# AtomGradient/swift-qwen3-tts

Hardware: AMD Instinct MI355X
Metric: codec_tokens_per_s (higher is better)
Workload: dtype bf16

## Files before the change

### swift-qwen3-tts_amd/csrc/debug_env.cc

```cpp
#include <atomic>
#include <cstdlib>
#include <mutex>

#include "kernels.h"

namespace q3 {

namespace {
std::mutex g_mu;
std::atomic<const DebugEnv*> g_env{nullptr};

bool flag(const char* name) { return std::getenv(name) != nullptr; }
int number(const char* name, int dflt) {
    const char* e = std::getenv(name);
    return e && *e ? std::atoi(e) : dflt;
}

const DebugEnv* read_env() {
    DebugEnv* d = new DebugEnv{};
    d->gemm_no_row_split = flag("Q3TTS_GEMM_NO_ROW_SPLIT");
    d->gemm_one_pair = flag("Q3TTS_GEMM_ONE_PAIR");
    d->no_tall_gemm = flag("Q3TTS_NO_TALL_GEMM");
    d->tall_shape = number("Q3TTS_TALL_SHAPE", 0);
    d->chunk_qsplit = number("Q3TTS_CHUNK_QSPLIT", 0);
    d->conv_no_pw = flag("Q3TTS_CONV_NO_PW");
    d->nt_off = std::getenv("Q3TTS_NT") && number("Q3TTS_NT", 1) == 0;
    d->serial_jobs = number("Q3TTS_SERIAL_JOBS", 0) != 0;
    d->fail_back_half = number("Q3TTS_TEST_FAIL_BACK_HALF", 0) != 0;
    d->no_prefix_cache = number("Q3TTS_NO_PREFIX_CACHE", 0) != 0;
    return d;
}
}

const DebugEnv& debug_env() {
    const DebugEnv* e = g_env.load(std::memory_order_acquire);
    if (!e) {
        std::lock_guard<std::mutex> lk(g_mu);
        e = g_env.load(std::memory_order_acquire);
        if (!e) {
            e = read_env();
            g_env.store(e, std::memory_order_release);
        }
    }
    return *e;
}

void debug_env_reload() {
    std::lock_guard<std::mutex> lk(g_mu);
    g_env.store(read_env(), std::memory_order_release);
}

}
```

### swift-qwen3-tts_amd/csrc/engine.cc

```cpp
#include "engine.h"

#include <algorithm>
#include <cctype>
#include <chrono>
#include <cmath>
#include <cstdio>
#include <deque>
#include <functional>
#include <thread>

#include "codec.h"
#include "frontend.h"

namespace q3 {

namespace {
std::string lower(const std::string& s) {
    std::string o = s;
    for (auto& c : o) c = char(std::tolower((unsigned char)c));
    return o;
}
const char* const kCodecRangeMsg =
    "Audio decoding failed: the codec decoder produced a non-finite waveform -- also on the fp32 matrix-core convolutions (the "
    "reference's range), which a row is re-decoded on when it leaves the fp16 range of the default two-plane kernels";
// ... 235 lines not shown
        compose_b_ = nullptr;
        if (!pass) {
            ws_bytes_ = align_up(b.off, 256);
            Q3_HIP(hipMalloc(reinterpret_cast<void**>(&ws_), ws_bytes_));
            Q3_HIP(hipMemset(ws_, 0, ws_bytes_));
        }
    }
    std::vector<int32_t> cbt((size_t)(Bm_));
    for (int i = 0; i < Bm_; ++i) cbt[size_t(i)] = i;
    Q3_HIP(hipMemcpy(cp_block_table_, cbt.data(), cbt.size() * 4, hipMemcpyHostToDevice));
}

GemmArgs Engine::gemm_args(const LinearW& L, const uint16_t* x, int M) const {
    GemmArgs a{};
    a.W = L.w;
    a.Wsb = L.sb;
    a.x = x;
    a.xMB = Mp_ / 16;
    a.M = M;
    a.Mpad = int(align_up(size_t(M), 16));
    a.N = L.Np;
    a.K = L.Kp;
    a.bias = L.bias;
    a.ss_ld = Mp_;
    return a;
}

void Engine::enqueue_layers(const StackW& s, Stream& w, int B, uint16_t* kpool, uint16_t* vpool, size_t layer_stride,
                            const int32_t* block_table, int max_pages, const int32_t* kv_len, const uint8_t* active,
                            int ss_count_in, int fixed_len, int chunk, const int32_t* chunk_n_prompt, int chunk_r_base) {
    const int H = s.hidden, MBL = Mp_ / 16, tiles = H / 16;
    const int M = B * (chunk > 1 ? chunk : 1);
    Q3_CHECK(M <= Mp_, 7, "internal error: chunk does not fit the activation buffers");
    const bool row_norm = M > 64;
    const bool prologue_qkv = H <= 2048 && !row_norm, prologue_mlp = H <= 2048 && !row_norm;
    const bool nt_off = debug_env().nt_off;
    const bool is_talker = &s == &m_->talker;
    const int ntw = is_talker && !nt_off ? 1 : 0;
    const int ntkv = ntw;
    auto norm_into_xn = [&](const uint16_t* nw, const float* ss, int ss_count) {
        NormRowsArgs n{};
        n.h = w.h; n.hMB = MBL; n.w = nw; n.eps = s.eps; n.out = w.xn; n.outMB = MBL; n.M = M; n.H = H;
        if (row_norm && H <= 2048) { n.ss_in = ss; n.ss_count = ss_count; n.ss_ld = Mp_; }
        launch_norm_rows(n, counted());
    };
    for (size_t l = 0; l < s.layers.size(); ++l) {
        const LayerW& L = s.layers[l];
        if (!prologue_qkv) norm_into_xn(L.ln1, w.ss_a, (l == 0) ? ss_count_in : tiles);
        GemmArgs q = gemm_args(L.qkv, prologue_qkv ? w.h : w.xn, M);
        q.epi = 0; q.y = w.qkv; q.ldy = w.ld_qkv; q.nt_weights = ntw;
        if (prologue_qkv) {
            q.norm_w = L.ln1; q.ss_in = w.ss_a; q.ss_count = (l == 0) ? ss_count_in : tiles; q.norm_dim = H; q.norm_eps = s.eps;
        }
        AttnArgs at{};
        at.qkv = w.qkv; at.ld = w.ld_qkv; at.qn_w = L.qn; at.kn_w = L.kn; at.eps = s.eps;
        at.rope_cos = s.rope_cos; at.rope_sin = s.rope_sin;
        at.kpool = kpool + l * layer_stride; at.vpool = vpool + l * layer_stride;
        at.block_table = block_table; at.max_pages = max_pages; at.kv_len = kv_len; at.active = active;
        at.out = w.ao; at.outMB = MBL; at.n_heads = s.n_heads; at.n_kv = s.n_kv; at.B = B;
        at.fixed_len = fixed_len; at.identity_pages = fixed_len >= 0 ? 1 : 0;
        at.chunk = chunk; at.chunk_n_prompt = chunk_n_prompt; at.chunk_r_base = chunk_r_base;
        at.scale = powf(float(kHeadDim), -0.5f);
        at.nt_kv = ntkv;
        launch_gemm_skinny(q, counted());
        launch_attn_decode(at, counted());
        GemmArgs o = gemm_args(L.o, w.ao, M);
        o.epi = 3; o.y = w.h; o.yMB = MBL; o.resid = 1; o.ss_out = w.ss_b; o.nt_weights = ntw;
        launch_gemm_skinny(o, counted());
        if (!prologue_mlp) norm_into_xn(L.ln2, w.ss_b, tiles);
        GemmArgs g = gemm_args(L.gateup, prologue_mlp ? w.h : w.xn, M);
        g.epi = 2; g.y = w.act; g.yMB = MBL; g.nt_weights = ntw;
        if (prologue_mlp) {
            g.norm_w = L.ln2; g.ss_in = w.ss_b; g.ss_count = tiles; g.norm_dim = H; g.norm_eps = s.eps;
        }
        launch_gemm_skinny(g, counted());
        GemmArgs d = gemm_args(L.down, w.act, M);
        d.epi = 3; d.y = w.h; d.yMB = MBL; d.resid = 1; d.ss_out = w.ss_a; d.nt_weights = ntw;
        launch_gemm_skinny(d, counted());
    }
}

void Engine::enqueue_talker_step(int B, bool with_head) {
    (void)with_head;
    enqueue_layers(m_->talker, tk_, B, kpool_, vpool_, kv_layer_stride_, block_table_, max_pages_, kv_len_, active_, 1, -1, 1, nullptr, 0);
}

void Engine::enqueue_cp_pass(int B, bool from_talker, int head, int cp_pos, bool projected) {
    const TalkerConfig& t = m_->cfg.talker;
    const int H = t.hidden_size, CH = m_->cp.hidden, MBL = Mp_ / 16;
    int ss_count = 1;
    auto talker_norm_into = [&](uint16_t* dst, float* ss_out) {
        NormRowsArgs n{};
        n.h = tk_.h; n.hMB = MBL; n.w = m_->talker.final_norm; n.eps = m_->talker.eps;
        n.out = dst; n.outMB = MBL; n.ss_out = ss_out; n.M = B; n.H = H;
        launch_norm_rows(n, counted());
    };
    if (m_->has_cp_proj && projected) {
        ss_count = CH / 16;
    } else if (m_->has_cp_proj) {
        if (from_talker) talker_norm_into(cp_x2_, nullptr);
        GemmArgs p = gemm_args(m_->cp_proj, from_talker ? cp_x2_ : cp_x_, B);
        p.epi = 3; p.y = cp_.h; p.yMB = MBL; p.resid = 0; p.ss_out = cp_.ss_a;
        launch_gemm_skinny(p, counted());
        ss_count = CH / 16;
    } else if (from_talker) {
        talker_norm_into(cp_.h, cp_.ss_a);
    }
    enqueue_layers(m_->cp, cp_, B, cp_kpool_, cp_vpool_, cp_kv_layer_stride_, cp_block_table_, 1, cp_len_, nullptr, ss_count, cp_pos, 1, nullptr, 0);
}

FrameEndArgs Engine::frame_end_args(int B) const {
    const TalkerConfig& t = m_->cfg.talker;
    FrameEndArgs fe{};
    fe.cur_codes = cur_codes_; fe.codec_emb = m_->codec_emb; fe.cp_emb = m_->cp_emb_dev;
    fe.trailing = trailing_; fe.n_trailing = n_trailing_; fe.trailing_idx = trailing_idx_; fe.Tmax = Tcap_;
    fe.tts_pad = tts_pad_; fe.h = tk_.h; fe.hMB = Mp_ / 16; fe.ss_out = tk_.ss_a; fe.H = t.hidden_size; fe.B = B; fe.groups = t.num_code_groups;
    fe.n_frames = n_frames_; fe.max_frames = max_frames_; fe.finished = finished_; fe.active = active_; fe.cp_len = cp_len_;
    fe.text_open = frame_text_open_; fe.starved = frame_text_open_ ? starved_ : nullptr;
    return fe;
}

void Engine::enqueue_frame(int B, const DebugOpts* dbg) {
    struct Count {
        Engine* e;
        int B;
        ~Count() { e->frame_launches_[B] = e->launches_; }
    } count{this, B};
    launches_ = 0;
    const TalkerConfig& t = m_->cfg.talker;
    const int H = t.hidden_size, V = t.vocab_size, Vc = t.cp.vocab_size, CH = t.cp.hidden_size;
    const int groups = t.num_code_groups, MBL = Mp_ / 16;
    stamp(0);
    enqueue_talker_step(B, true);
    stamp(1);
    uint16_t* next_x = m_->has_cp_proj ? cp_x_ : cp_.h;
    float* next_ss = m_->has_cp_proj ? nullptr : cp_.ss_a;
    const bool pair = 2 * B <= Mp_;
    {
        GemmArgs hd = gemm_args(m_->codec_head, tk_.h, B);
        hd.epi = 0; hd.y = tk_.logits; hd.ldy = tk_.ld_logits;
        hd.norm_w = m_->talker.final_norm; hd.ss_in = tk_.ss_a; hd.ss_count = H / 16; hd.norm_dim = H; hd.norm_eps = m_->talker.eps;
        bool rode = false;
        if (pair) {
            NormRowsArgs n{};
            n.h = tk_.h; n.hMB = MBL; n.w = m_->talker.final_norm; n.eps = m_->talker.eps;
            n.out = next_x; n.outMB = MBL; n.ss_out = next_ss; n.M = B; n.H = H;
            rode = launch_gemm_skinny_with_norm_rows(hd, n, st_);
            if (rode) ++launches_;
            else launch_norm_rows(n, counted());
        }
        if (!rode) launch_gemm_skinny(hd, counted());
    }
    SamplerArgs sa{};
    sa.logits = tk_.logits; sa.ldl = tk_.ld_logits; sa.V = V; sa.sp = sp_dev_; sa.is_talker = 1;
    sa.suppress_lo = V - 1024; sa.suppress_hi = V; sa.eos_id = t.codec_eos_token_id;
    sa.seen = seen_; sa.cb = 0; sa.n_frames = n_frames_; sa.max_frames = max_frames_;
    sa.finished = finished_; sa.active = active_; sa.kv_len = kv_len_; sa.advance = 1; sa.advance_gate = active_;
    sa.cur_codes = cur_codes_; sa.codes = codes_; sa.Fmax = Fcap_;
    sa.forced = dbg ? forced_dev_ : nullptr; sa.forced_frames = dbg ? dbg->frames : 0;
    sa.sampled = dbg ? sampled_dev_ : nullptr;
    sa.emb = m_->codec_emb; sa.emb_ld = H; sa.next_MB = MBL; sa.H = H; sa.B = B;
    if (pair) {
        sa.next_x = next_x; sa.next_row0 = B; sa.next_ss = next_ss ? next_ss + B : nullptr;
    } else {
        sa.next_x = m_->has_cp_proj ? cp_x_ : cp_x2_; sa.next_ss = m_->has_cp_proj ? nullptr : cp_ss2_;
    }
    sa.logits_dump = (dbg && dbg->talker_logits) ? tl_dump_ : nullptr; sa.dump_ld = V; sa.dump_off = 0;
    sa.row_key = frame_row_key_;
    if (pair) {
        launch_sampler(sa, counted());
// ... 2565 lines not shown
    qkv.grow(size_t(rows) * ld);
    w.grow(2 * kHeadDim);
    rope.grow(2 * tab);
    kp.grow(pool);
    vp.grow(pool);
    ot.grow(size_t(Mp) * odim);
    ol.grow(size_t(rows) * odim);
    ints.grow(size_t(B) * (2 + d.max_pages));
    act.grow(size_t(B));
    int32_t *kv_len = ints, *n_prompt = kv_len + B, *bt = n_prompt + B;
    Q3_HIP(hipMemset(ints, 0, size_t(B) * (2 + d.max_pages) * 4));
    Q3_HIP(hipMemcpy(qkv, d.qkv, size_t(rows) * ld * 2, hipMemcpyHostToDevice));
    Q3_HIP(hipMemcpy(w, d.qn_w, kHeadDim * 2, hipMemcpyHostToDevice));
    Q3_HIP(hipMemcpy(w + kHeadDim, d.kn_w, kHeadDim * 2, hipMemcpyHostToDevice));
    Q3_HIP(hipMemcpy(rope, d.rope_cos, tab * 2, hipMemcpyHostToDevice));
    Q3_HIP(hipMemcpy(rope + tab, d.rope_sin, tab * 2, hipMemcpyHostToDevice));
    Q3_HIP(hipMemcpy(kp, d.kpool, pool * 2, hipMemcpyHostToDevice));
    Q3_HIP(hipMemcpy(vp, d.vpool, pool * 2, hipMemcpyHostToDevice));
    if (d.kv_len) Q3_HIP(hipMemcpy(kv_len, d.kv_len, size_t(B) * 4, hipMemcpyHostToDevice));
    if (d.chunk_n_prompt) Q3_HIP(hipMemcpy(n_prompt, d.chunk_n_prompt, size_t(B) * 4, hipMemcpyHostToDevice));
    if (d.block_table) Q3_HIP(hipMemcpy(bt, d.block_table, size_t(B) * d.max_pages * 4, hipMemcpyHostToDevice));
    if (d.active) Q3_HIP(hipMemcpy(act, d.active, size_t(B), hipMemcpyHostToDevice));
    Q3_HIP(hipMemset(ot, 0xff, size_t(Mp) * odim * 2));
    AttnArgs at{};
    at.qkv = qkv; at.ld = ld; at.qn_w = w; at.kn_w = w + kHeadDim; at.eps = d.eps;
    at.rope_cos = rope; at.rope_sin = rope + tab;
    at.kpool = kp; at.vpool = vp;
    at.block_table = bt; at.max_pages = d.max_pages; at.kv_len = kv_len; at.active = d.active ? (const uint8_t*)act : nullptr;
    at.out = ot; at.outMB = Mp / 16; at.n_heads = d.n_heads; at.n_kv = d.n_kv; at.B = B;
    at.scale = d.scale;
    at.fixed_len = d.fixed_len; at.identity_pages = d.identity_pages ? 1 : 0;
    at.chunk = d.chunk; at.chunk_n_prompt = d.chunk_n_prompt ? n_prompt : nullptr; at.chunk_r_base = d.chunk_r_base;
    at.nt_kv = d.nt_kv ? 1 : 0;
    launch_attn_decode(at, st_);
    Q3_HIP(hipGetLastError());
    launch_untile_rows(ot, Mp / 16, ol, odim, rows, odim, st_);
    Q3_HIP(hipStreamSynchronize(st_));
    Q3_HIP(hipMemcpy(d.out, ol, size_t(rows) * odim * 2, hipMemcpyDeviceToHost));
    Q3_HIP(hipMemcpy(d.kpool, kp, pool * 2, hipMemcpyDeviceToHost));
    Q3_HIP(hipMemcpy(d.vpool, vp, pool * 2, hipMemcpyDeviceToHost));
}

void Engine::debug_gemm_check(q3tts_gemm_debug& d, GemmArgs& ga, NormRowsArgs& na) {
    static const uint16_t dummy16 = 0;
    static const uint32_t dummy32 = 0;
    d.rode = d.tall = d.tall_shape = d.split = d.mbw = d.nw = d.ch = d.np = d.gx = d.ntw = 0;
    Q3_CHECK(d.mode == 0 || d.mode == 1, 3, "debug_gemm: unknown mode");
    const bool rider = d.mode == 1 || d.rider_M > 0;
    if (rider) {
        Q3_CHECK(d.rider_M >= 1 && d.rider_MB >= 1 && d.rider_MB <= 64 && d.rider_M <= 16 * d.rider_MB, 3, "debug_gemm: rider rows out of range");
        Q3_CHECK(d.rider_H >= 128 && d.rider_H <= 4096 && d.rider_H % 128 == 0, 3, "debug_gemm: rider_H must be a multiple of 128 up to 4096");
        Q3_CHECK(d.geometry_only || (d.rider_h && d.rider_w && d.rider_out), 3, "debug_gemm: null rider argument");
        if (d.rider_ss_in) Q3_CHECK(d.rider_ss_count >= 1 && d.rider_ss_count <= 256, 3, "debug_gemm: at most 256 partial sums of squares per rider row");
        na.hMB = na.outMB = d.rider_MB; na.eps = d.rider_eps; na.M = d.rider_M; na.H = d.rider_H;
        na.ss_count = d.rider_ss_in ? d.rider_ss_count : 0; na.ss_ld = 16 * d.rider_MB;
    }
    if (d.mode == 1) return;
    Q3_CHECK(d.epi == 0 || d.epi == 2 || d.epi == 3, 3, "debug_gemm: unknown epilogue");
    Q3_CHECK(d.M >= 1 && d.M <= 1024, 3, "debug_gemm: M out of range");
    Q3_CHECK(d.K >= 128 && d.K <= 8192 && d.K % 128 == 0, 3, "debug_gemm: K must be a multiple of 128 up to 8192");
    Q3_CHECK(d.N >= 8 && d.N <= 65536 && d.N % (d.epi == 2 ? 8 : 16) == 0, 3, "debug_gemm: N must be a multiple of 16 (epi 2: of 8)");
    const int Mp = int(align_up(size_t(d.M), 16));
    const bool tiled = d.epi != 0 || d.y_tiled;
    Q3_CHECK(d.xMB <= 64 && 16 * d.xMB >= Mp && d.yMB <= 64 && 16 * d.yMB >= Mp && d.ss_ld >= Mp && d.ss_ld <= 4096, 3,
             "debug_gemm: allocation smaller than the padded batch");
    Q3_CHECK(d.y_cols >= d.N && d.y_cols <= d.N + 1024 && d.y_cols % (tiled ? 128 : 8) == 0, 3, "debug_gemm: y_cols");
// ... 96 lines not shown
        for (int part = 0; part < (d.epi == 2 ? 2 : 1); ++part) {
            const void* W = part ? d.W_up : d.W;
            if (d.quant) {
                dWq.grow(size_t(d.N) * d.K / 8);
                Q3_HIP(hipMemcpy(dWq, W, size_t(d.N) * d.K / 8 * 4, hipMemcpyHostToDevice));
                up16(dsc, part ? d.scales_up : d.scales, size_t(d.N) * d.K / 64);
                up16(dbi, part ? d.biases_up : d.biases, size_t(d.N) * d.K / 64);
                launch_tile_int4(dWq, dsc, dbi, d.N, d.K, dWt, dsb, KC, 0, 1, st_, rpt, 8 * part);
            } else {
                up16(dsrc, static_cast<const uint16_t*>(W), size_t(d.N) * d.K);
                launch_tile_weights(dsrc, d.N, d.K, reinterpret_cast<uint16_t*>(static_cast<uint8_t*>(dWt)), KC, 0, 1, st_, rpt, 8 * part);
            }
            Q3_HIP(hipStreamSynchronize(st_));
        }
        if (d.bias) up16(dbias, d.bias, size_t(d.N));
        if (d.norm) {
            up16(dnw, d.norm_w, size_t(d.K));
            dssi.grow(size_t(d.ss_count) * d.ss_ld);
            Q3_HIP(hipMemcpy(dssi, d.ss_in, size_t(d.ss_count) * d.ss_ld * 4, hipMemcpyHostToDevice));
        }
        if (d.ss_out) {
            dsso.grow(n_ss_out);
            Q3_HIP(hipMemcpy(dsso, d.ss_out, n_ss_out * 4, hipMemcpyHostToDevice));
        }
        ga.W = reinterpret_cast<const uint16_t*>(static_cast<uint8_t*>(dWt));
        ga.Wsb = d.quant ? static_cast<uint32_t*>(dsb) : nullptr;
        ga.x = dx; ga.y = dy;
        ga.bias = d.bias ? static_cast<uint16_t*>(dbias) : nullptr;
        ga.norm_w = d.norm ? static_cast<uint16_t*>(dnw) : nullptr;
        ga.ss_in = d.norm ? static_cast<float*>(dssi) : nullptr;
        ga.ss_out = d.ss_out ? static_cast<float*>(dsso) : nullptr;
    }
    bool launched = true;
    if (d.mode == 1) {
        launch_norm_rows(na, st_);
    } else if (rider) {
        launched = launch_gemm_skinny_with_norm_rows(ga, na, st_);
        Q3_CHECK(launched == (d.rode != 0), 7, "debug_gemm: the rider launch disagrees with gemm_norm_rows_rides");
    } else {
        launch_gemm_skinny(ga, st_);
    }
    Q3_HIP(hipGetLastError());
    Q3_HIP(hipStreamSynchronize(st_));
    if (!launched) return;
    if (d.mode == 0) {
        if (tiled) {
            tmp.resize(size_t(yrows) * d.y_cols);
            Q3_HIP(hipMemcpy(tmp.data(), dy, tmp.size() * 2, hipMemcpyDeviceToHost));
            host_untile(tmp, d.y, yrows, d.y_cols);
        } else {
            Q3_HIP(hipMemcpy(d.y, dy, size_t(yrows) * d.y_cols * 2, hipMemcpyDeviceToHost));
        }
        if (d.ss_out) Q3_HIP(hipMemcpy(d.ss_out, dsso, n_ss_out * 4, hipMemcpyDeviceToHost));
    }
    if (rider) {
        tmp.resize(size_t(rrows) * d.rider_H);
        Q3_HIP(hipMemcpy(tmp.data(), rout, tmp.size() * 2, hipMemcpyDeviceToHost));
        host_untile(tmp, d.rider_out, rrows, d.rider_H);
        if (d.rider_ss_out) Q3_HIP(hipMemcpy(d.rider_ss_out, rsso, size_t(rrows) * 4, hipMemcpyDeviceToHost));
    }
}

static void check_caller_codes(const CodecW& w, const int32_t* codes, const int32_t* n_frames, int batch, int max_frames) {
    for (int b = 0; b < batch; ++b)
        for (int f = 0; f < n_frames[b]; ++f) {
            const int32_t* c = codes + (size_t(b) * max_frames + f) * 16;
// ... 669 lines not shown
```

### swift-qwen3-tts_amd/csrc/kernels.h

```cpp
#pragma once
#include <hip/hip_runtime.h>

#include <cstdint>

namespace q3 {

struct DebugEnv {
    bool gemm_no_row_split;
    bool gemm_one_pair;
    bool no_tall_gemm;
    int tall_shape;
    int chunk_qsplit;
    bool conv_no_pw;
    bool nt_off;
    bool serial_jobs;
    bool fail_back_half;
    bool no_prefix_cache;
};
const DebugEnv& debug_env();
void debug_env_reload();

constexpr int kPageTokens = 64;
constexpr int kHeadDim = 128;

struct NormRowsArgs {
    const uint16_t* h;
    int hMB;
    const uint16_t* w;
    float eps;
    uint16_t* out;
    int outMB;
    float* ss_out;
    int M, H;
    const float* ss_in;
    int ss_count, ss_ld;
};
void launch_norm_rows(const NormRowsArgs& a, hipStream_t st);

struct GemmArgs {
    const uint16_t* W;
    const uint32_t* Wsb;
    const uint16_t* x;
    int xMB;
    int M, Mpad, N, K;
    int epi;
    uint16_t* y;
    int ldy;
    int y_tiled, yMB;
    const uint16_t* bias;
    int act_silu;
    const uint16_t* norm_w;
    const float* ss_in;
    int ss_count, ss_ld, norm_dim;
    float norm_eps;
    int nt_weights;
    int resid;
    float* ss_out;
};
void launch_gemm_skinny(const GemmArgs& a, hipStream_t st);
struct SkinnyGeom {
    bool tall;
    int split, mbw;
    int nw, ch, np;
    int gx;
    bool ntw;
};
SkinnyGeom skinny_geometry(const GemmArgs& a);
bool launch_gemm_skinny_with_norm_rows(const GemmArgs& a, const NormRowsArgs& n, hipStream_t st);
bool gemm_norm_rows_rides(const GemmArgs& a, const NormRowsArgs& n);
bool launch_gemm_tall(const GemmArgs& a, hipStream_t st);
bool gemm_tall_takes(const GemmArgs& a);
int gemm_tall_shape(const GemmArgs& a);


struct AttnArgs {
    const uint16_t* qkv;
    int ld;
    const uint16_t* qn_w;
    const uint16_t* kn_w;
    float eps;
    const uint16_t* rope_cos;
    const uint16_t* rope_sin;
    uint16_t* kpool;
// ... 171 lines not shown
```

### swift-qwen3-tts_amd/csrc/kernels/gemm_decode.hip

```cpp
#include "../common.h"
#include "../kernels.h"
#include "row_jobs.h"

namespace q3 {

namespace {

#include "gemm_body.inc"

template <int MB, int EPI, int NW, int CH, bool NORM, bool QUANT, int NP = 1, bool NTW = false>
__global__ __launch_bounds__(NW * 64) void gemm_skinny_kernel(GemmArgs a) {
    __builtin_amdgcn_s_setprio(3);
    gemm_skinny_body<MB, EPI, NW, CH, NORM, QUANT, NP, NTW>(a, blockIdx.x, blockIdx.y * MB);
}

struct GemmSideArgs {
    GemmArgs g;
    NormRowsArgs n;
    int tiles;
};
template <int MB, int CH, bool QUANT>
__global__ __launch_bounds__(512) void gemm_skinny_side_kernel(GemmSideArgs s) {
    __builtin_amdgcn_s_setprio(3);
    if (int(blockIdx.x) >= s.tiles) {
// ... 10 lines not shown
    const dim3 grid(g.gx, g.split);
#define Q3_GEMM(NWv, CHv) \
    hipLaunchKernelGGL((gemm_skinny_kernel<MB, EPI, NWv, CHv, NORM, QUANT, 1, NTW>), grid, dim3(NWv * 64), 0, st, a)
    if constexpr (MB == 4 && !NORM && !NTW) {
        if (g.ch == 0 && g.np == 2) { hipLaunchKernelGGL((gemm_skinny_kernel<4, EPI, 8, 0, false, QUANT, 2, false>), grid, dim3(512), 0, st, a); return; }
        if (g.ch == 0 && g.np == 4) { hipLaunchKernelGGL((gemm_skinny_kernel<4, EPI, 8, 0, false, QUANT, 4, false>), grid, dim3(512), 0, st, a); return; }
    }
    if constexpr (EPI == 2 && MB <= 2) {
        if (g.np > 1) {
#define Q3_GEMM_NP(CHv, NPv) hipLaunchKernelGGL((gemm_skinny_kernel<MB, 2, 8, CHv, NORM, QUANT, NPv, NTW>), grid, dim3(512), 0, st, a)
            if (g.ch == 1) { if (g.np == 2) Q3_GEMM_NP(1, 2); else Q3_GEMM_NP(1, 3); }
            else { if (g.np == 2) Q3_GEMM_NP(2, 2); else Q3_GEMM_NP(2, 3); }
#undef Q3_GEMM_NP
            return;
        }
    }
    if (g.nw == 4) {
        Q3_GEMM(4, 1);
    } else {
        switch (g.ch) {
            case 1: Q3_GEMM(8, 1); break;
            case 2: Q3_GEMM(8, 2); break;
            case 3: Q3_GEMM(8, 3); break;
            case 6: Q3_GEMM(8, 6); break;
            default: Q3_GEMM(8, 0); break;
        }
    }
#undef Q3_GEMM
}

template <int EPI, bool NORM, bool QUANT>
void launch_q(const GemmArgs& a, hipStream_t st) {
    const SkinnyGeom g = skinny_geometry(a);
    if (g.ntw) {
        if (g.mbw == 1) launch_mb<1, EPI, NORM, QUANT, true>(a, g, st);
        else launch_mb<2, EPI, NORM, QUANT, true>(a, g, st);
        return;
    }
    switch (g.mbw) {
        case 1: launch_mb<1, EPI, NORM, QUANT, false>(a, g, st); break;
        case 2: launch_mb<2, EPI, NORM, QUANT, false>(a, g, st); break;
        case 3: launch_mb<3, EPI, NORM, QUANT, false>(a, g, st); break;
        case 4: launch_mb<4, EPI, NORM, QUANT, false>(a, g, st); break;
        default: throw Error(3, "gemm_skinny: more than 4 row blocks per workgroup");
    }
}

template <int EPI, bool NORM>
void launch_epi(const GemmArgs& a, hipStream_t st) {
    if (a.Wsb) launch_q<EPI, NORM, true>(a, st);
    else launch_q<EPI, NORM, false>(a, st);
}

}

SkinnyGeom skinny_geometry(const GemmArgs& a) {
    SkinnyGeom g{};
    if (gemm_tall_takes(a)) {
        g.tall = true;
        return g;
    }
    const DebugEnv& env = debug_env();
    const bool norm = a.norm_w != nullptr;
    const int MBt = (a.Mpad + 15) / 16;
    const bool no_split = env.gemm_no_row_split;
    int tiles = a.N / 16;
    if (a.epi == 2) {
        const int t8 = a.N / 8;
        tiles = t8 > 512 ? (t8 + 2) / 3 : (t8 > 256 ? (t8 + 1) / 2 : t8);
    }
    int split = 1;
    if (!no_split) {
        if (MBt % 4 == 0 && tiles * 4 <= 256) split = 4;
        else if (MBt % 2 == 0 && tiles * 2 <= 256) split = 2;
        const int cap = norm ? 2 : 4;
        while (MBt / split > cap || MBt % split != 0) ++split;
    }
    while (MBt / split > 4 || MBt % split != 0) ++split;
    g.split = split;
    g.mbw = MBt / split;
    g.ntw = a.nt_weights && g.mbw <= 2;
    const int KC = a.K / 128;
    g.nw = KC <= 4 ? 4 : 8;
    g.ch = (KC + g.nw - 1) / g.nw;
    g.np = 1;
    const int t = a.epi == 2 ? a.N / 8 : a.N / 16;
    g.gx = t;
    bool shaped = false;
    if (g.mbw == 4 && !norm && !g.ntw && !env.gemm_one_pair && g.nw == 8 && t >= 64) {
        g.np = (((t + 3) / 4) * split <= 128) ? 2 : 4;
        g.ch = 0;
        g.gx = (t + g.np - 1) / g.np;
        shaped = true;
    }
    if (!shaped && a.epi == 2 && g.mbw <= 2) {
        const int np = env.gemm_one_pair ? 1 : (t > 512 ? 3 : (t > 256 ? 2 : 1));
        if (g.nw == 8 && (g.ch == 1 || g.ch == 2) && np > 1) {
            g.np = np;
            g.gx = (t + np - 1) / np;
            shaped = true;
        }
    }
    if (!shaped) {
        if (g.nw == 4) g.ch = 1;
        else if (g.ch != 1 && g.ch != 2 && g.ch != 3 && g.ch != 6) g.ch = 0;
    }
    return g;
}

bool gemm_norm_rows_rides(const GemmArgs& a, const NormRowsArgs& n) {
    if (a.epi != 0 || !a.norm_w || a.nt_weights || n.M <= 0 || n.H > 4096) return false;
    if (a.K % 128 != 0 || a.N % 16 != 0) return false;
    const SkinnyGeom g = skinny_geometry(a);
    return !(g.tall || g.nw != 8 || g.np != 1 || (g.ch != 1 && g.ch != 2) || g.mbw < 1 || g.mbw > 2 || g.ntw);
}

bool launch_gemm_skinny_with_norm_rows(const GemmArgs& a, const NormRowsArgs& n, hipStream_t st) {
    if (!gemm_norm_rows_rides(a, n)) return false;
    const SkinnyGeom g = skinny_geometry(a);
    Q3_CHECK(a.ss_in && a.ss_count >= 1 && a.ss_ld >= a.Mpad && a.xMB * 16 >= a.Mpad, 3, "gemm_skinny: norm prologue needs sums of squares");
    const int tiles = g.gx;
    const dim3 grid(tiles + n.M, g.split), block(512);
    const GemmSideArgs s{a, n, tiles};
    const bool q = a.Wsb != nullptr;
#define Q3_SIDE(MBv, CHv)                                                                              \
    do {                                                                                               \
        if (q) hipLaunchKernelGGL((gemm_skinny_side_kernel<MBv, CHv, true>), grid, block, 0, st, s);   \
        else hipLaunchKernelGGL((gemm_skinny_side_kernel<MBv, CHv, false>), grid, block, 0, st, s);    \
// ... 25 lines not shown
```

### swift-qwen3-tts_amd/csrc/kernels/gemm_prefill.hip

```cpp
#include <cstdlib>

#include "../common.h"
#include "../kernels.h"

namespace q3 {

namespace {

using u32x4 = __attribute__((ext_vector_type(4))) uint32_t;
__device__ __forceinline__ f32x4 mfma16t(const u32x4& a, const u32x4& b, f32x4 c) {
    return __builtin_amdgcn_mfma_f32_16x16x32_bf16(__builtin_bit_cast(bf16x8, a), __builtin_bit_cast(bf16x8, b), c, 0, 0, 0);
}
__device__ __forceinline__ float silu_t(float v) { return v / (1.0f + __expf(-v)); }

struct Stage {
    int w, kc, half;
};

template <int GM, int GN, int WM, int WN, int EPI, int D>
__global__ __launch_bounds__(64 * GM * GN, 2) void gemm_tall_kernel(GemmArgs a, int nphase) {
    constexpr int NWV = GM * GN;
    constexpr int TMB = GM * WM, TNT = GN * WN;
    constexpr int FR = (TMB + TNT) * 2;
    constexpr int LV = FR / NWV;
// ... 138 lines not shown
                for (int j = 0; j < 4; ++j) {
                    float h0 = lo_bf(yw[j]), h1 = hi_bf(yw[j]);
                    if (a.resid) {
                        h0 = rbf(lo_bf(hw[j]) + h0);
                        h1 = rbf(hi_bf(hw[j]) + h1);
                    }
                    ss += h0 * h0;
                    ss += h1 * h1;
                    ow[j] = pack_bf(h0, h1);
                }
                const float other = __shfl_xor(ss, 32, 64);
                if (mine) {
                    *reinterpret_cast<uint4*>(hp) = make_uint4(ow[0], ow[1], ow[2], ow[3]);
                    if (pc == 0 && a.ss_out) a.ss_out[(size_t)otile * a.ss_ld + m] = ss + other;
                }
            }
        }
    }
}

template <int GM, int GN, int WM, int WN, int D>
void launch_shape(const GemmArgs& a, int n_tiles, int nphase, hipStream_t st) {
    const dim3 grid((n_tiles + GN * WN - 1) / (GN * WN), ((a.Mpad >> 4) + GM * WM - 1) / (GM * WM)), block(64 * GM * GN);
    switch (a.epi) {
        case 0: hipLaunchKernelGGL((gemm_tall_kernel<GM, GN, WM, WN, 0, D>), grid, block, 0, st, a, nphase); break;
        case 2: hipLaunchKernelGGL((gemm_tall_kernel<GM, GN, WM, WN, 2, D>), grid, block, 0, st, a, nphase); break;
        default: hipLaunchKernelGGL((gemm_tall_kernel<GM, GN, WM, WN, 3, D>), grid, block, 0, st, a, nphase); break;
    }
}

}

bool gemm_tall_takes(const GemmArgs& a) {
    if (debug_env().no_tall_gemm || a.Mpad <= 64 || a.Wsb || a.norm_w || a.bias || a.act_silu) return false;
    if (a.epi != 0 && a.epi != 2 && a.epi != 3) return false;
    if (a.epi == 0 && a.N % 16 != 0) return false;
    return true;
}

int gemm_tall_shape(const GemmArgs& a) {
    const int n_tiles = a.epi == 2 ? a.N / 8 : a.N / 16;
    const int MBt = a.Mpad / 16;
    const int force = debug_env().tall_shape;
    auto wgs = [&](int tm, int tn) { return ((MBt + tm - 1) / tm) * ((n_tiles + tn - 1) / tn); };
    int shape = wgs(8, 4) >= 192 ? 2 : 3;
    if (force == 2 || force == 3) shape = force;
    return shape;
}

bool launch_gemm_tall(const GemmArgs& a, hipStream_t st) {
    if (!gemm_tall_takes(a)) return false;
    const int KC = a.K / 128;
    const int nphase = KC <= 4 ? 4 : 8;
    const int n_tiles = a.epi == 2 ? a.N / 8 : a.N / 16;
    if (gemm_tall_shape(a) == 2) launch_shape<2, 2, 4, 2, 4>(a, n_tiles, nphase, st);
    else launch_shape<2, 2, 2, 2, 8>(a, n_tiles, nphase, st);
    return true;
}

}
```

### swift-qwen3-tts_amd/csrc/kernels/gemm_body.inc

```
__device__ __forceinline__ f32x4 mfma16(const uint4& a, const uint4& b, f32x4 c) {
    bf16x8 av, bv;
    __builtin_memcpy(&av, &a, 16);
    __builtin_memcpy(&bv, &b, 16);
    return __builtin_amdgcn_mfma_f32_16x16x32_bf16(av, bv, c, 0, 0, 0);
}

__device__ __forceinline__ float silu_f(float v) { return v / (1.0f + __expf(-v)); }

__device__ __forceinline__ uint4 norm8(const uint4& hx, const uint4& wx, float rstd) {
    const uint32_t hw[4] = {hx.x, hx.y, hx.z, hx.w}, ww[4] = {wx.x, wx.y, wx.z, wx.w};
    uint32_t o[4];
#pragma unroll
    for (int j = 0; j < 4; ++j) {
        const float n0 = rbf(lo_bf(hw[j]) * rstd), n1 = rbf(hi_bf(hw[j]) * rstd);
        o[j] = pack_bf(n0 * lo_bf(ww[j]), n1 * hi_bf(ww[j]));
    }
    return make_uint4(o[0], o[1], o[2], o[3]);
}

__device__ __forceinline__ void dequant_chunk(const uint4& qw, uint32_t sb, uint4 (&out)[4]) {
    const float sc = lo_bf(sb), bi = hi_bf(sb);
    const uint32_t w[4] = {qw.x, qw.y, qw.z, qw.w};
#pragma unroll
    for (int i = 0; i < 4; ++i) {
// ... 18 lines not shown
    __shared__ float ssp_s[NORM ? 8 : 1][NORM ? 16 * MB : 1];

    const int lane = threadIdx.x & 63;
    const int wave = threadIdx.x >> 6;
    const int KC = a.K >> 7;

    f32x4 acc[NT][MB];
#pragma unroll
    for (int t = 0; t < NT; ++t)
#pragma unroll
        for (int mb = 0; mb < MB; ++mb) acc[t][mb] = f32x4{0.f, 0.f, 0.f, 0.f};

    const uint4* Wt = reinterpret_cast<const uint4*>(a.W);
    const uint4* Xt = reinterpret_cast<const uint4*>(a.x);

    constexpr int kSsIter = NORM ? (16 * MB * 8 + NW * 64 - 1) / (NW * 64) : 1;
    float sst[kSsIter][16];
    if constexpr (NORM) {
        const int rows = 16 * MB;
#pragma unroll
        for (int it = 0; it < kSsIter; ++it) {
            const int idx = (threadIdx.x + it * NW * 64) % (rows * 8);
            const int row = idx % rows, part = idx / rows;
            const float* sp = a.ss_in + 16 * mb0 + row;
#pragma unroll
            for (int u = 0; u < 16; ++u) {
                const int j = part + 8 * u;
                sst[it][u] = sp[(size_t)(j < a.ss_count ? j : 0) * a.ss_ld];
            }
        }
        __builtin_amdgcn_sched_barrier(0);
    }

    constexpr int CHR = CH > 0 ? CH : 1;
    constexpr int WL = QUANT ? 1 : 4;
    uint4 wf[CHR][NT][WL];
    uint32_t wsb[CHR][NT];
    auto load_w = [&](int c, int kc) {
#pragma unroll
        for (int t = 0; t < NT; ++t) {
            const int tt = tile * NT + t;
            const size_t blk = (size_t)(tt < n_tiles ? tt : n_tiles - 1) * KC + kc;
            if constexpr (QUANT) {
                wf[c][t][0] = ld16<NTW>(Wt + blk * 64 + lane);
                wsb[c][t] = a.Wsb[blk * 64 + lane];
            } else {
                const uint4* wp = Wt + blk * 256 + lane;
#pragma unroll
                for (int i = 0; i < 4; ++i) wf[c][t][i] = ld16<NTW>(wp + i * 64);
            }
        }
    };

    constexpr int kWRegs = CH * NT * (QUANT ? 5 : 16);
    constexpr int kRoom = (((MB == 1 && !NORM) ? 200 : 176) - kWRegs) / (MB * 16);
    constexpr int kCap = (MB == 1 && !NORM) ? 6 : 3;
    constexpr int XG0 = (CH == 0) ? 0 : (kRoom < 1 ? 1 : (kRoom > kCap ? (CH < kCap ? CH : kCap) : (kRoom < CH ? kRoom : CH)));
    constexpr int XG = (MB == 2 && NORM && CH == 2 && NT == 1 && EPI == 0) ? 1 : XG0;
    uint4 xr[XG > 0 ? XG : 1][MB][4];
    uint4 nwr[(NORM && XG > 0) ? XG : 1][4];
#pragma unroll
    for (int ph = 0; ph < 2; ++ph) {
        if (ph == 1) __builtin_amdgcn_sched_barrier(0);
        if ((ph == 0) != NORM) {
    if constexpr (CH > 0) {
#pragma unroll
            for (int c = 0; c < CH; ++c) {
                const int kl = wave + c * NW;
                load_w(c, kl < KC ? kl : 0);
            }
        }
        } else {
    if constexpr (XG > 0) {
#pragma unroll
        for (int c = 0; c < XG; ++c) {
            const int kl = wave + c * NW;
            const int kc = kl < KC ? kl : 0;
            if constexpr (NORM) {
                const uint4* np = reinterpret_cast<const uint4*>(a.norm_w + kc * 128 + 32 * (lane >> 4));
#pragma unroll
                for (int i = 0; i < 4; ++i) nwr[c][i] = np[i];
            }
#pragma unroll
            for (int mb = 0; mb < MB; ++mb) {
                const uint4* xp = Xt + ((size_t)(kc * a.xMB + mb0 + mb) * 4) * 64 + lane;
#pragma unroll
                for (int i = 0; i < 4; ++i) xr[c][mb][i] = xp[i * 64];
            }
        }
    }
        }
    }
    __builtin_amdgcn_sched_barrier(0);
    uint4 hv_pre = make_uint4(0, 0, 0, 0);
    if constexpr (EPI == 3 && NT == 1) {
        if (a.resid && threadIdx.x < 32 * MB) {
            const int o = threadIdx.x, mb = o >> 5, b = (o >> 1) & 15, p = o & 1;
            hv_pre = *reinterpret_cast<const uint4*>(a.y + act_tiled_offset(16 * (mb0 + mb) + b, tile * 16 + 8 * p, a.yMB));
        }
    }

    float rstd[MB];
    if constexpr (NORM) {
        const int rows = 16 * MB;
#pragma unroll
        for (int it = 0; it < kSsIter; ++it) {
            const int idx = threadIdx.x + it * NW * 64;
            if (idx < rows * 8) {
// ... 31 lines not shown
        }
        uint4 nw[4];
        if constexpr (NORM) {
            if (nwpre) {
#pragma unroll
                for (int i = 0; i < 4; ++i) nw[i] = nwpre[i];
            } else {
                const uint4* np = reinterpret_cast<const uint4*>(a.norm_w + kc * 128 + 32 * (lane >> 4));
#pragma unroll
                for (int i = 0; i < 4; ++i) nw[i] = np[i];
            }
        }
#pragma unroll
        for (int mb = 0; mb < MB; ++mb) {
            uint4 xf[4];
            if (xpre) {
#pragma unroll
                for (int i = 0; i < 4; ++i) xf[i] = xpre[mb][i];
            } else {
                const uint4* xp = Xt + ((size_t)(kc * a.xMB + mb0 + mb) * 4) * 64 + lane;
#pragma unroll
                for (int i = 0; i < 4; ++i) xf[i] = xp[i * 64];
            }
            if constexpr (NORM) {
#pragma unroll
                for (int i = 0; i < 4; ++i) xf[i] = norm8(xf[i], nw[i], rstd[mb]);
            }
#pragma unroll
            for (int t = 0; t < NT; ++t)
#pragma unroll
                for (int i = 0; i < 4; ++i) acc[t][mb] = mfma16(w[t][i], xf[i], acc[t][mb]);
        }
    };
    if constexpr (CH > 0) {
#pragma unroll
        for (int g0 = 0; g0 < CH; g0 += XG) {
            if (g0 > 0) {
#pragma unroll
                for (int c = 0; c < XG; ++c) {
                    if (g0 + c < CH) {
                        const int kl = wave + (g0 + c) * NW;
                        const int kc = kl < KC ? kl : 0;
                        if constexpr (NORM) {
                            const uint4* np = reinterpret_cast<const uint4*>(a.norm_w + kc * 128 + 32 * (lane >> 4));
#pragma unroll
                            for (int i = 0; i < 4; ++i) nwr[c][i] = np[i];
                        }
#pragma unroll
                        for (int mb = 0; mb < MB; ++mb) {
                            const uint4* xp = Xt + ((size_t)(kc * a.xMB + mb0 + mb) * 4) * 64 + lane;
#pragma unroll
                            for (int i = 0; i < 4; ++i) xr[c][mb][i] = xp[i * 64];
                        }
                    }
                }
            }
#pragma unroll
            for (int c = 0; c < XG; ++c) {
                if (g0 + c < CH) {
                    const int kl = wave + (g0 + c) * NW;
                    if (kl < KC) chunk(kl, g0 + c, xr[c], NORM ? nwr[c] : nullptr);
                }
            }
        }
    } else {
        for (int kl = wave; kl < KC; kl += NW) {
            load_w(0, kl);
// ... 96 lines not shown
```

Measured before the change: 10290.

## Route paired two-token chunk steps through skinny GEMMs with fused norm prologue

For two-token chunk passes with a fixed length and 128 padded rows, the layer stack now skips the separate row-norm kernels and the tall GEMM path. Norm is fused as a prologue into the skinny GEMMs instead. The skinny geometry also gains a four-row-block mode for the norm-fused gate/up GEMM, using a 512-thread kernel with three column pairs and non-temporal weights. The goal is fewer launches and intermediate round-trips for the pair form. The cost is larger per-workgroup register and LDS pressure in the four-block kernel, plus new debug env knobs.

```diff
diff --git a/swift-qwen3-tts_amd/csrc/debug_env.cc b/swift-qwen3-tts_amd/csrc/debug_env.cc
--- a/swift-qwen3-tts_amd/csrc/debug_env.cc
+++ b/swift-qwen3-tts_amd/csrc/debug_env.cc
@@ -21,6 +21,8 @@
     d->gemm_no_row_split = flag("Q3TTS_GEMM_NO_ROW_SPLIT");
     d->gemm_one_pair = flag("Q3TTS_GEMM_ONE_PAIR");
     d->no_tall_gemm = flag("Q3TTS_NO_TALL_GEMM");
+    d->gemm_norm_two_blocks = flag("Q3TTS_GEMM_NORM_TWO_BLOCKS");
+    d->pair_form = number("Q3TTS_PAIR_FORM", 0);
     d->tall_shape = number("Q3TTS_TALL_SHAPE", 0);
     d->chunk_qsplit = number("Q3TTS_CHUNK_QSPLIT", 0);
     d->conv_no_pw = flag("Q3TTS_CONV_NO_PW");
diff --git a/swift-qwen3-tts_amd/csrc/engine.cc b/swift-qwen3-tts_amd/csrc/engine.cc
--- a/swift-qwen3-tts_amd/csrc/engine.cc
+++ b/swift-qwen3-tts_amd/csrc/engine.cc
@@ -291,7 +291,9 @@
     const int H = s.hidden, MBL = Mp_ / 16, tiles = H / 16;
     const int M = B * (chunk > 1 ? chunk : 1);
     Q3_CHECK(M <= Mp_, 7, "internal error: chunk does not fit the activation buffers");
-    const bool row_norm = M > 64;
+    const bool pair_skinny = chunk == 2 && fixed_len >= 0 && align_up(size_t(M), 16) == 128 && debug_env().pair_form != 1 &&
+                             !s.layers.empty() && s.layers.front().qkv.sb == nullptr;
+    const bool row_norm = M > 64 && !pair_skinny;
     const bool prologue_qkv = H <= 2048 && !row_norm, prologue_mlp = H <= 2048 && !row_norm;
     const bool nt_off = debug_env().nt_off;
     const bool is_talker = &s == &m_->talker;
@@ -307,7 +309,7 @@
         const LayerW& L = s.layers[l];
         if (!prologue_qkv) norm_into_xn(L.ln1, w.ss_a, (l == 0) ? ss_count_in : tiles);
         GemmArgs q = gemm_args(L.qkv, prologue_qkv ? w.h : w.xn, M);
-        q.epi = 0; q.y = w.qkv; q.ldy = w.ld_qkv; q.nt_weights = ntw;
+        q.epi = 0; q.y = w.qkv; q.ldy = w.ld_qkv; q.nt_weights = ntw; q.no_tall = pair_skinny;
         if (prologue_qkv) {
             q.norm_w = L.ln1; q.ss_in = w.ss_a; q.ss_count = (l == 0) ? ss_count_in : tiles; q.norm_dim = H; q.norm_eps = s.eps;
         }
@@ -324,17 +326,17 @@
         launch_gemm_skinny(q, counted());
         launch_attn_decode(at, counted());
         GemmArgs o = gemm_args(L.o, w.ao, M);
-        o.epi = 3; o.y = w.h; o.yMB = MBL; o.resid = 1; o.ss_out = w.ss_b; o.nt_weights = ntw;
+        o.epi = 3; o.y = w.h; o.yMB = MBL; o.resid = 1; o.ss_out = w.ss_b; o.nt_weights = ntw; o.no_tall = pair_skinny;
         launch_gemm_skinny(o, counted());
         if (!prologue_mlp) norm_into_xn(L.ln2, w.ss_b, tiles);
         GemmArgs g = gemm_args(L.gateup, prologue_mlp ? w.h : w.xn, M);
-        g.epi = 2; g.y = w.act; g.yMB = MBL; g.nt_weights = ntw;
+        g.epi = 2; g.y = w.act; g.yMB = MBL; g.nt_weights = ntw; g.no_tall = pair_skinny;
         if (prologue_mlp) {
             g.norm_w = L.ln2; g.ss_in = w.ss_b; g.ss_count = tiles; g.norm_dim = H; g.norm_eps = s.eps;
         }
         launch_gemm_skinny(g, counted());
         GemmArgs d = gemm_args(L.down, w.act, M);
-        d.epi = 3; d.y = w.h; d.yMB = MBL; d.resid = 1; d.ss_out = w.ss_a; d.nt_weights = ntw;
+        d.epi = 3; d.y = w.h; d.yMB = MBL; d.resid = 1; d.ss_out = w.ss_a; d.nt_weights = ntw; d.no_tall = pair_skinny;
         launch_gemm_skinny(d, counted());
     }
 }
@@ -394,7 +396,7 @@
     stamp(1);
     uint16_t* next_x = m_->has_cp_proj ? cp_x_ : cp_.h;
     float* next_ss = m_->has_cp_proj ? nullptr : cp_.ss_a;
-    const bool pair = 2 * B <= Mp_;
+    const bool pair = 2 * B <= Mp_ && !(debug_env().pair_form == 3 && 2 * B > 64);
     {
         GemmArgs hd = gemm_args(m_->codec_head, tk_.h, B);
         hd.epi = 0; hd.y = tk_.logits; hd.ldy = tk_.ld_logits;
diff --git a/swift-qwen3-tts_amd/csrc/kernels.h b/swift-qwen3-tts_amd/csrc/kernels.h
--- a/swift-qwen3-tts_amd/csrc/kernels.h
+++ b/swift-qwen3-tts_amd/csrc/kernels.h
@@ -9,6 +9,8 @@
     bool gemm_no_row_split;
     bool gemm_one_pair;
     bool no_tall_gemm;
+    bool gemm_norm_two_blocks;
+    int pair_form;
     int tall_shape;
     int chunk_qsplit;
     bool conv_no_pw;
@@ -49,6 +51,7 @@
     int y_tiled, yMB;
     const uint16_t* bias;
     int act_silu;
+    int no_tall;
     const uint16_t* norm_w;
     const float* ss_in;
     int ss_count, ss_ld, norm_dim;
diff --git a/swift-qwen3-tts_amd/csrc/kernels/gemm_decode.hip b/swift-qwen3-tts_amd/csrc/kernels/gemm_decode.hip
--- a/swift-qwen3-tts_amd/csrc/kernels/gemm_decode.hip
+++ b/swift-qwen3-tts_amd/csrc/kernels/gemm_decode.hip
@@ -66,6 +66,14 @@
 template <int EPI, bool NORM, bool QUANT>
 void launch_q(const GemmArgs& a, hipStream_t st) {
     const SkinnyGeom g = skinny_geometry(a);
+    if constexpr (EPI == 2 && NORM) {
+        if (g.mbw == 4 && g.np == 3) {
+            const dim3 grid(g.gx, g.split);
+            if (g.ntw) hipLaunchKernelGGL((gemm_skinny_kernel<4, 2, 8, 2, true, QUANT, 3, true>), grid, dim3(512), 0, st, a);
+            else hipLaunchKernelGGL((gemm_skinny_kernel<4, 2, 8, 2, true, QUANT, 3, false>), grid, dim3(512), 0, st, a);
+            return;
+        }
+    }
     if (g.ntw) {
         if (g.mbw == 1) launch_mb<1, EPI, NORM, QUANT, true>(a, g, st);
         else launch_mb<2, EPI, NORM, QUANT, true>(a, g, st);
@@ -98,6 +106,9 @@
     const bool norm = a.norm_w != nullptr;
     const int MBt = (a.Mpad + 15) / 16;
     const bool no_split = env.gemm_no_row_split;
+    const int KCn = a.K / 128;
+    const bool four = norm && a.epi == 2 && MBt == 4 && a.N / 8 > 512 && KCn > 8 && KCn <= 16 && !no_split && !env.gemm_one_pair &&
+                      !env.gemm_norm_two_blocks;
     int tiles = a.N / 16;
     if (a.epi == 2) {
         const int t8 = a.N / 8;
@@ -107,13 +118,13 @@
     if (!no_split) {
         if (MBt % 4 == 0 && tiles * 4 <= 256) split = 4;
         else if (MBt % 2 == 0 && tiles * 2 <= 256) split = 2;
-        const int cap = norm ? 2 : 4;
+        const int cap = norm && !four ? 2 : 4;
         while (MBt / split > cap || MBt % split != 0) ++split;
     }
     while (MBt / split > 4 || MBt % split != 0) ++split;
     g.split = split;
     g.mbw = MBt / split;
-    g.ntw = a.nt_weights && g.mbw <= 2;
+    g.ntw = a.nt_weights && (g.mbw <= 2 || four);
     const int KC = a.K / 128;
     g.nw = KC <= 4 ? 4 : 8;
     g.ch = (KC + g.nw - 1) / g.nw;
@@ -127,7 +138,7 @@
         g.gx = (t + g.np - 1) / g.np;
         shaped = true;
     }
-    if (!shaped && a.epi == 2 && g.mbw <= 2) {
+    if (!shaped && a.epi == 2 && (g.mbw <= 2 || four)) {
         const int np = env.gemm_one_pair ? 1 : (t > 512 ? 3 : (t > 256 ? 2 : 1));
         if (g.nw == 8 && (g.ch == 1 || g.ch == 2) && np > 1) {
             g.np = np;
diff --git a/swift-qwen3-tts_amd/csrc/kernels/gemm_prefill.hip b/swift-qwen3-tts_amd/csrc/kernels/gemm_prefill.hip
--- a/swift-qwen3-tts_amd/csrc/kernels/gemm_prefill.hip
+++ b/swift-qwen3-tts_amd/csrc/kernels/gemm_prefill.hip
@@ -194,7 +194,7 @@
 }
 
 bool gemm_tall_takes(const GemmArgs& a) {
-    if (debug_env().no_tall_gemm || a.Mpad <= 64 || a.Wsb || a.norm_w || a.bias || a.act_silu) return false;
+    if (debug_env().no_tall_gemm || a.no_tall || a.Mpad <= 64 || a.Wsb || a.norm_w || a.bias || a.act_silu) return false;
     if (a.epi != 0 && a.epi != 2 && a.epi != 3) return false;
     if (a.epi == 0 && a.N % 16 != 0) return false;
     return true;
```

Result: slower. 10010 (-2.7%).

## Ring-buffer weight tiles in skinny GEMM for three-tile SiLU epilogue variant

Applied to the files above, without the earlier changes.

For the NT==3, EPI==2 skinny GEMM instantiation, only two output tiles' worth of weight fragments are held in registers. The third tile's weights are loaded into the freed slot after the first tile's MFMAs, and x fragments are pre-normalized once and reused across tiles. The aim is to cut register pressure, so occupancy or the x-staging depth can improve, at the cost of exposing the third tile's weight-load latency mid-loop. The debug paths also clear stale HIP errors before launches.

```diff
diff --git a/swift-qwen3-tts_amd/csrc/engine.cc b/swift-qwen3-tts_amd/csrc/engine.cc
--- a/swift-qwen3-tts_amd/csrc/engine.cc
+++ b/swift-qwen3-tts_amd/csrc/engine.cc
@@ -3026,6 +3026,7 @@
     at.fixed_len = d.fixed_len; at.identity_pages = d.identity_pages ? 1 : 0;
     at.chunk = d.chunk; at.chunk_n_prompt = d.chunk_n_prompt ? n_prompt : nullptr; at.chunk_r_base = d.chunk_r_base;
     at.nt_kv = d.nt_kv ? 1 : 0;
+    (void)hipGetLastError();
     launch_attn_decode(at, st_);
     Q3_HIP(hipGetLastError());
     launch_untile_rows(ot, Mp / 16, ol, odim, rows, odim, st_);
@@ -3188,6 +3189,7 @@
         ga.ss_out = d.ss_out ? static_cast<float*>(dsso) : nullptr;
     }
     bool launched = true;
+    (void)hipGetLastError();
     if (d.mode == 1) {
         launch_norm_rows(na, st_);
     } else if (rider) {
diff --git a/swift-qwen3-tts_amd/csrc/kernels/gemm_body.inc b/swift-qwen3-tts_amd/csrc/kernels/gemm_body.inc
--- a/swift-qwen3-tts_amd/csrc/kernels/gemm_body.inc
+++ b/swift-qwen3-tts_amd/csrc/kernels/gemm_body.inc
@@ -74,24 +74,27 @@
         __builtin_amdgcn_sched_barrier(0);
     }
 
+    constexpr bool RING_T = (NT == 3 && EPI == 2 && CH > 0);
+    constexpr int NTS = RING_T ? 2 : NT;
     constexpr int CHR = CH > 0 ? CH : 1;
     constexpr int WL = QUANT ? 1 : 4;
-    uint4 wf[CHR][NT][WL];
-    uint32_t wsb[CHR][NT];
+    uint4 wf[CHR][NTS][WL];
+    uint32_t wsb[CHR][NTS];
+    auto load_wt = [&](int c, int kc, int t, int s) {
+        const int tt = tile * NT + t;
+        const size_t blk = (size_t)(tt < n_tiles ? tt : n_tiles - 1) * KC + kc;
+        if constexpr (QUANT) {
+            wf[c][s][0] = ld16<NTW>(Wt + blk * 64 + lane);
+            wsb[c][s] = a.Wsb[blk * 64 + lane];
+        } else {
+            const uint4* wp = Wt + blk * 256 + lane;
+#pragma unroll
+            for (int i = 0; i < 4; ++i) wf[c][s][i] = ld16<NTW>(wp + i * 64);
+        }
+    };
     auto load_w = [&](int c, int kc) {
 #pragma unroll
-        for (int t = 0; t < NT; ++t) {
-            const int tt = tile * NT + t;
-            const size_t blk = (size_t)(tt < n_tiles ? tt : n_tiles - 1) * KC + kc;
-            if constexpr (QUANT) {
-                wf[c][t][0] = ld16<NTW>(Wt + blk * 64 + lane);
-                wsb[c][t] = a.Wsb[blk * 64 + lane];
-            } else {
-                const uint4* wp = Wt + blk * 256 + lane;
-#pragma unroll
-                for (int i = 0; i < 4; ++i) wf[c][t][i] = ld16<NTW>(wp + i * 64);
-            }
-        }
+        for (int t = 0; t < NTS; ++t) load_wt(c, kc, t, t);
     };
 
     constexpr int kWRegs = CH * NT * (QUANT ? 5 : 16);
@@ -99,8 +102,11 @@
     constexpr int kCap = (MB == 1 && !NORM) ? 6 : 3;
     constexpr int XG0 = (CH == 0) ? 0 : (kRoom < 1 ? 1 : (kRoom > kCap ? (CH < kCap ? CH : kCap) : (kRoom < CH ? kRoom : CH)));
     constexpr int XG = (MB == 2 && NORM && CH == 2 && NT == 1 && EPI == 0) ? 1 : XG0;
+    constexpr int XGT = (RING_T && MB == 2 && NORM && CH == 2) ? 1 : XG;
+    static_assert(!RING_T || XG == CH, "the tile ring keeps the x fragments of every chunk");
     uint4 xr[XG > 0 ? XG : 1][MB][4];
-    uint4 nwr[(NORM && XG > 0) ? XG : 1][4];
+    uint4 xst[XGT < XG ? MB : 1][4];
+    uint4 nwr[(NORM && XG > 0) ? XGT : 1][4];
 #pragma unroll
     for (int ph = 0; ph < 2; ++ph) {
         if (ph == 1) __builtin_amdgcn_sched_barrier(0);
@@ -115,7 +121,7 @@
         } else {
     if constexpr (XG > 0) {
 #pragma unroll
-        for (int c = 0; c < XG; ++c) {
+        for (int c = 0; c < XGT; ++c) {
             const int kl = wave + c * NW;
             const int kc = kl < KC ? kl : 0;
             if constexpr (NORM) {
@@ -213,7 +219,69 @@
                 for (int i = 0; i < 4; ++i) acc[t][mb] = mfma16(w[t][i], xf[i], acc[t][mb]);
         }
     };
-    if constexpr (CH > 0) {
+    if constexpr (RING_T) {
+        if constexpr (NORM) {
+#pragma unroll
+            for (int c = 0; c < XGT; ++c)
+#pragma unroll
+                for (int mb = 0; mb < MB; ++mb)
+#pragma unroll
+                    for (int i = 0; i < 4; ++i) xr[c][mb][i] = norm8(xr[c][mb][i], nwr[c][i], rstd[mb]);
+            if constexpr (XGT < CH) {
+                __builtin_amdgcn_sched_barrier(0);
+                const int kl = wave + NW;
+                const int kc = kl < KC ? kl : 0;
+                const uint4* np = reinterpret_cast<const uint4*>(a.norm_w + kc * 128 + 32 * (lane >> 4));
+#pragma unroll
+                for (int i = 0; i < 4; ++i) nwr[0][i] = np[i];
+#pragma unroll
+                for (int mb = 0; mb < MB; ++mb) {
+                    const uint4* xp = Xt + ((size_t)(kc * a.xMB + mb0 + mb) * 4) * 64 + lane;
+#pragma unroll
+                    for (int i = 0; i < 4; ++i) xst[mb][i] = xp[i * 64];
+                }
+                __builtin_amdgcn_sched_barrier(0);
+            }
+        }
+#pragma unroll
+        for (int t = 0; t < NT; ++t) {
+            const int s = t % NTS;
+#pragma unroll
+            for (int c = 0; c < CH; ++c) {
+                const int kl = wave + c * NW;
+                if constexpr (NORM && XGT < CH) {
+                    if (t == 0 && c == 1) {
+#pragma unroll
+                        for (int mb = 0; mb < MB; ++mb)
+#pragma unroll
+                            for (int i = 0; i < 4; ++i) xr[1][mb][i] = norm8(xst[mb][i], nwr[0][i], rstd[mb]);
+                    }
+                }
+                if (kl < KC) {
+                    uint4 w[4];
+                    if constexpr (QUANT) {
+                        dequant_chunk(wf[c][s][0], wsb[c][s], w);
+                    } else {
+#pragma unroll
+                        for (int i = 0; i < 4; ++i) w[i] = wf[c][s][i];
+                    }
+#pragma unroll
+                    for (int mb = 0; mb < MB; ++mb)
+#pragma unroll
+                        for (int i = 0; i < 4; ++i) acc[t][mb] = mfma16(w[i], xr[c][mb][i], acc[t][mb]);
+                }
+            }
+            if (t + NTS < NT) {
+                __builtin_amdgcn_sched_barrier(0);
+#pragma unroll
+                for (int c = 0; c < CH; ++c) {
+                    const int kl = wave + c * NW;
+                    load_wt(c, kl < KC ? kl : 0, t + NTS, s);
+                }
+                __builtin_amdgcn_sched_barrier(0);
+            }
+        }
+    } else if constexpr (CH > 0) {
 #pragma unroll
         for (int g0 = 0; g0 < CH; g0 += XG) {
             if (g0 > 0) {
```

After: 10310 before, 10120 after. 0.981x the previous value.
